# fschmid56/EfficientAT

Hardware: NVIDIA H100
Metric: clips/sec (10s@32kHz) mn10_as fwd+bwd (higher is better)
Workload: dtype f32

## Files before the change

efficientat_b200/csrc/pw_tma.cu:

```cuda
#include <cstdlib>

#include "tma_common.cuh"

namespace {
using namespace tc;
using namespace tma;

constexpr int BM = 128;
constexpr int BN_MAX = 128;
constexpr int A_TILE = BM * 128;
constexpr int kThreads = 416;
constexpr int kFirstCons = 4, kTmaWarp = 12, kConsThreads = 256;
constexpr int STG_BYTES = 16 * 128;

struct TmaParams {
  int M, N, K;
  int BN, n_tiles, m_tiles, k_blocks, r_blocks;
  int bnp;
  int stages, wres;
  int stg_bufs;
  int wpre;
  int n_samples, tps, tile_rps;
  int wdyn;
  uint32_t stage_bytes, off_w, off_stg, off_f, off_bar;
  int kpad;
  const float* in_scale; const float* in_shift; const float* gate; int in_act; int rps;
  const float* scale; const float* shift;
  double* stat_sum; double* stat_sq;
};

template <int NP>
__device__ __forceinline__ void mma_pieces(float (&d)[NP][16], uint64_t da, uint64_t db) {
#pragma unroll
  for (int pc = 0; pc < NP; ++pc) wgmma_n32<0, 0>(d[pc], da, db + (uint64_t)(pc * 256));
}

template <int EPI, int XACT, int NP>
__global__ void __launch_bounds__(kThreads, 1)
pw_tma_kernel(const __grid_constant__ CUtensorMap mapA, const __grid_constant__ CUtensorMap mapW,
              const __grid_constant__ CUtensorMap mapC, const __grid_constant__ CUtensorMap mapR, const TmaParams p) {
  extern __shared__ __align__(1024) unsigned char smem[];
  unsigned char* s_w = smem + p.off_w;
  unsigned char* s_stg = smem + p.off_stg;
  float* s_isc = reinterpret_cast<float*>(smem + p.off_f);
  float* s_ish = s_isc + p.kpad;
  float* s_shift = s_ish + p.kpad;
  float* s_stat = s_shift + p.bnp;
  uint64_t* bars = reinterpret_cast<uint64_t*>(smem + p.off_bar);
  const int S = p.stages;
  const uint32_t bar_full = smem_u32(bars), bar_ready = bar_full + 8 * S, bar_empty = bar_ready + 8 * S;
  const uint32_t bar_wfull = bar_empty + 8 * S;

  const int warp = threadIdx.x >> 5, lane = threadIdx.x & 31;
  if (threadIdx.x == 0) {
    for (int s = 0; s < S; ++s) { mbar_init(bar_full + 8 * s, 1); mbar_init(bar_ready + 8 * s, 4); mbar_init(bar_empty + 8 * s, 2); }
    mbar_init(bar_wfull, 1);
    asm volatile("fence.mbarrier_init.release.cluster;" ::: "memory");
    asm volatile("prefetch.tensormap [%0];" ::"l"(reinterpret_cast<uint64_t>(&mapA)) : "memory");
    asm volatile("prefetch.tensormap [%0];" ::"l"(reinterpret_cast<uint64_t>(&mapW)) : "memory");
    asm volatile("prefetch.tensormap [%0];" ::"l"(reinterpret_cast<uint64_t>(&mapC)) : "memory");
  }
  if (XACT >= 0) {
    for (int i = threadIdx.x; i < p.kpad; i += kThreads) {
      s_isc[i] = i < p.K ? p.in_scale[i] : 0.f;
      s_ish[i] = i < p.K ? p.in_shift[i] : 0.f;
    }
  }
  for (int i = threadIdx.x; i < 16 * p.bnp; i += kThreads) s_stat[i] = 0.f;
  fence_proxy_async();
  __syncthreads();

  const int total_tiles = p.m_tiles * p.n_tiles;
  constexpr int BN = 32 * NP;
  const int kb_total = p.k_blocks + p.r_blocks;
  const uint32_t w_tile = (uint32_t)BN * 128u;
  const uint32_t stage_base = smem_u32(smem);
  int nt = blockIdx.x / p.m_tiles, mt = blockIdx.x - nt * p.m_tiles;
  auto next_tile = [&]() { mt += gridDim.x; while (mt >= p.m_tiles) { mt -= p.m_tiles; ++nt; } };
  auto split_tile = [&](int m, int& bs, int& jt) { if (p.n_samples == 1) { bs = 0; jt = m; } else { bs = m / p.tps; jt = m - bs * p.tps; } };

  if (warp == kTmaWarp) {
    if (lane == 0) {
      int s = 0, s_prev = 0, cur_nt = -1;
      uint32_t ph = 0, ph_prev = 0;
      bool first = true;
      for (int t = blockIdx.x; t < total_tiles; t += gridDim.x) {
        int bs, jt;
        split_tile(mt, bs, jt);
        const int m0 = jt * BM, n0 = nt * BN;
        const int wb = p.wdyn ? bs : 0;
        const int wkey = nt * p.n_samples + wb;
        if (p.wres && wkey != cur_nt) {
          if (!first) mbar_wait(bar_empty + 8 * s_prev, ph_prev);
          mbar_expect_tx(bar_wfull, (uint32_t)p.k_blocks * w_tile);
          for (int kb = 0; kb < p.k_blocks; ++kb)
            tma_load_3d(&mapW, bar_wfull, smem_u32(s_w) + (uint32_t)kb * w_tile, kb * (p.wpre ? 2 * KB : KB), n0, wb);
          cur_nt = wkey;
        }
        next_tile();
        for (int kb = 0; kb < kb_total; ++kb) {
          mbar_wait(bar_empty + 8 * s, ph ^ 1u);
          const uint32_t dst = stage_base + (uint32_t)s * p.stage_bytes;
          if (kb < p.k_blocks) {
            mbar_expect_tx(bar_full + 8 * s, A_TILE + (p.wres ? 0u : w_tile));
            tma_load_3d(&mapA, bar_full + 8 * s, dst, kb * KB, m0, bs);
            if (!p.wres) tma_load_3d(&mapW, bar_full + 8 * s, dst + A_TILE, kb * (p.wpre ? 2 * KB : KB), n0, wb);
          } else {
            mbar_expect_tx(bar_full + 8 * s, A_TILE);
            tma_load_3d(&mapR, bar_full + 8 * s, dst, n0 + (kb - p.k_blocks) * KB, m0, bs);
          }
          s_prev = s; ph_prev = ph; first = false;
          if (++s == S) { s = 0; ph ^= 1u; }
        }
      }
    }
    __syncwarp();
  } else if (warp < kFirstCons) {
    const int ft = threadIdx.x;
    int s = 0, cur_nt = -1;
    uint32_t ph = 0, wphase = 0;
    const bool fold = EPI != 0 && p.scale != nullptr;
    auto do_fix_w = [&](unsigned char* w, int kb, int n0) {
      const int lg = pair_lg(p.K - kb * KB);
      if (fold) {
        if (lg == 2) fix_w<2, true>(w, ft, BN, p.scale, n0, p.N);
        else fix_w<1, true>(w, ft, BN, p.scale, n0, p.N);
      } else {
        if (lg == 2) fix_w<2, false>(w, ft, BN, nullptr, n0, p.N);
        else fix_w<1, false>(w, ft, BN, nullptr, n0, p.N);
      }
    };
    for (int t = blockIdx.x; t < total_tiles; t += gridDim.x) {
      int bs, jt;
      split_tile(mt, bs, jt);
      const int n0 = nt * BN;
      const int rows_valid = min(BM, p.tile_rps - jt * BM);
      const int wkey = nt * p.n_samples + (p.wdyn ? bs : 0);
      if (p.wres && wkey != cur_nt) {
        mbar_wait(bar_wfull, wphase);
        wphase ^= 1u;
        if (!p.wpre)
          for (int kb = 0; kb < p.k_blocks; ++kb) do_fix_w(s_w + (size_t)kb * w_tile, kb, n0);
        cur_nt = wkey;
      }
      next_tile();
      int b0 = 0, off0 = 0;
      if (p.gate != nullptr) { const int m0 = bs * p.tile_rps + jt * BM; b0 = m0 / p.rps; off0 = m0 - b0 * p.rps; }
      for (int kb = 0; kb < kb_total; ++kb) {
        mbar_wait(bar_full + 8 * s, ph);
        unsigned char* tile = smem + (size_t)s * p.stage_bytes;
        if (kb >= p.k_blocks) {
          fix_a<2, -1>(tile, ft, BM, nullptr, nullptr, 0, nullptr, 0, 0, 1, 0);
        } else {
          const int lg = pair_lg(p.K - kb * KB);
          const int k = kb * KB + (ft & ((1 << lg) - 1)) * 8;
          if (lg == 2) fix_a<2, XACT>(tile, ft, rows_valid, s_isc, s_ish, k, p.gate, off0, b0, p.rps, p.K);
          else fix_a<1, XACT>(tile, ft, rows_valid, s_isc, s_ish, k, p.gate, off0, b0, p.rps, p.K);
          if (!p.wres && !p.wpre) do_fix_w(tile + A_TILE, kb, n0);
        }
        fence_proxy_async();
        __syncwarp();
        if (lane == 0) mbar_arrive(bar_ready + 8 * s);
        if (++s == S) { s = 0; ph ^= 1u; }
      }
    }
  } else {
    const int cw = warp - kFirstCons;
    const int g = cw >> 2;
    const int wq = cw & 3;
    const int ctid = threadIdx.x - kFirstCons * 32;
    unsigned char* stg = s_stg + (size_t)cw * p.stg_bufs * STG_BYTES;
    const int bnp = p.bnp;
    float* my_stat = s_stat + cw * 2 * bnp;
    const bool do_stats = EPI == 0 && p.stat_sum != nullptr;
    const uint64_t desc0 = gmma_desc(0);
    const uint64_t wres0 = desc0 + (smem_u32(s_w) >> 4);
    const uint32_t w_tile16 = w_tile >> 4;
    float csum[NP], csq[NP];
#pragma unroll
    for (int c = 0; c < NP; ++c) { csum[c] = 0.f; csq[c] = 0.f; }
    int cur_nt = -1, cb = 0, s = 0;
    uint32_t ph = 0;
    auto flush_stats = [&](int nt_old) {
#pragma unroll
      for (int c = 0; c < NP; ++c) { my_stat[c * 32 + lane] = csum[c]; my_stat[bnp + c * 32 + lane] = csq[c]; csum[c] = 0.f; csq[c] = 0.f; }
      asm volatile("bar.sync 1, 256;" ::: "memory");
      for (int e = ctid; e < BN; e += kConsThreads) {
        const int n = nt_old * BN + e;
        float a = 0.f, b = 0.f;
#pragma unroll
        for (int w = 0; w < 8; ++w) { a += s_stat[w * 2 * bnp + e]; b += s_stat[w * 2 * bnp + bnp + e]; }
        if (n < p.N) { atomicAdd(p.stat_sum + n, (double)a); atomicAdd(p.stat_sq + n, (double)b); }
      }
      asm volatile("bar.sync 1, 256;" ::: "memory");
    };
    for (int t = blockIdx.x; t < total_tiles; t += gridDim.x) {
      int bs, jt;
      split_tile(mt, bs, jt);
      const int m0 = jt * BM, n0 = nt * BN;
      if (nt != cur_nt) {
        if (do_stats && cur_nt >= 0) flush_stats(cur_nt);
        if (EPI != 0) {
          asm volatile("bar.sync 2, 256;" ::: "memory");
          for (int e = ctid; e < BN; e += kConsThreads) s_shift[e] = (p.shift != nullptr && n0 + e < p.N) ? p.shift[n0 + e] : 0.f;
          asm volatile("bar.sync 2, 256;" ::: "memory");
        }
        cur_nt = nt;
      }
      next_tile();
      float acc[NP][16];
#pragma unroll
      for (int c = 0; c < NP; ++c)
#pragma unroll
        for (int i = 0; i < 16; ++i) acc[c][i] = 0.f;
      int pend = -1;
      auto release = [&](int st) {
        asm volatile("bar.sync %0, 128;" ::"r"(3 + g) : "memory");
        if (ctid == g * 128) mbar_arrive(bar_empty + 8 * st);
      };
      const int fr = lane >> 2, fc = 2 * (lane & 3);
      for (int kb = 0; kb < kb_total; ++kb) {
        mbar_wait(bar_ready + 8 * s, ph);
        const uint32_t sa = stage_base + (uint32_t)s * p.stage_bytes;
        if (kb < p.k_blocks) {
          const uint64_t a_hi = desc0 + ((sa + (uint32_t)g * 8192u) >> 4), a_lo = a_hi + 4;
          const uint64_t w_hi = p.wres ? wres0 + (uint32_t)kb * w_tile16 : desc0 + ((sa + A_TILE) >> 4);
          const uint64_t w_lo = w_hi + 4;
          wgmma_fence();
#pragma unroll
          for (int j = 0; j < 2; ++j) {
            const uint64_t ko = (uint64_t)(j * 2);
            mma_pieces<NP>(acc, a_hi + ko, w_hi + ko);
            mma_pieces<NP>(acc, a_lo + ko, w_hi + ko);
            mma_pieces<NP>(acc, a_hi + ko, w_lo + ko);
          }
          wgmma_commit();
          wgmma_wait<1>();
          if (pend >= 0) release(pend);
          pend = s;
        } else {
          wgmma_wait<0>();
#pragma unroll
          for (int c = 0; c < NP; ++c) wgmma_fence_regs(acc[c]);
          if (pend >= 0) { release(pend); pend = -1; }
          const int jr = kb - p.k_blocks;
          const unsigned char* tile = smem + (size_t)s * p.stage_bytes;
          const int r0 = g * 64 + wq * 16 + fr;
#pragma unroll
          for (int c = 0; c < NP; ++c) {
            if (c == jr) {
#pragma unroll
              for (int j = 0; j < 4; ++j) {
#pragma unroll
                for (int h = 0; h < 2; ++h) {
                  const int r = r0 + 8 * h;
                  const uint32_t e = (uint32_t)fc * 2;
                  const __nv_bfloat162 hi = *reinterpret_cast<const __nv_bfloat162*>(tile + swz(r, j) + e);
                  const __nv_bfloat162 lo = *reinterpret_cast<const __nv_bfloat162*>(tile + swz(r, 4 + j) + e);
                  const float2 fh = __bfloat1622float2(hi), fl = __bfloat1622float2(lo);
                  acc[c][4 * j + 2 * h] += fh.x + fl.x;
                  acc[c][4 * j + 2 * h + 1] += fh.y + fl.y;
                }
              }
            }
          }
          release(s);
        }
        if (++s == S) { s = 0; ph ^= 1u; }
      }
      if (pend >= 0) {
        wgmma_wait<0>();
        release(pend);
      }
#pragma unroll
      for (int c = 0; c < NP; ++c) wgmma_fence_regs(acc[c]);
      const int row0 = m0 + g * 64 + wq * 16;
      const int rows_left = min(16, p.tile_rps - row0);
#pragma unroll
      for (int c = 0; c < NP; ++c) {
        if (c * 32 < BN && n0 + c * 32 < p.N) {
          unsigned char* buf = stg + (size_t)cb * STG_BYTES;
          if (p.stg_bufs == 2) { cb ^= 1; if (lane == 0) tma_wait_read<1>(); }
          else if (lane == 0) tma_wait_read<0>();
          __syncwarp();
#pragma unroll
          for (int j = 0; j < 4; ++j) {
            const int cc = 8 * j + fc;
            float2 v0 = make_float2(acc[c][4 * j], acc[c][4 * j + 1]), v1 = make_float2(acc[c][4 * j + 2], acc[c][4 * j + 3]);
            if (EPI != 0) {
              const float2 sh = *reinterpret_cast<const float2*>(s_shift + c * 32 + cc);
              v0.x = act_out<EPI>(v0.x + sh.x); v0.y = act_out<EPI>(v0.y + sh.y);
              v1.x = act_out<EPI>(v1.x + sh.x); v1.y = act_out<EPI>(v1.y + sh.y);
            }
            const uint32_t co = (uint32_t)(((cc >> 2) << 4) + (cc & 3) * 4);
            *reinterpret_cast<float2*>(buf + fr * 128 + (co ^ ((fr & 7) << 4))) = v0;
            *reinterpret_cast<float2*>(buf + (fr + 8) * 128 + (co ^ (((fr + 8) & 7) << 4))) = v1;
          }
          if (do_stats) {
            __syncwarp();
            float s1 = 0.f, s2 = 0.f;
            const int cj = lane >> 2, ci = lane & 3;
            for (int r = 0; r < rows_left; ++r) {
              const float x = *reinterpret_cast<const float*>(buf + r * 128 + ((cj ^ (r & 7)) << 4) + ci * 4);
              s1 += x; s2 = fmaf(x, x, s2);
            }
            csum[c] += s1; csq[c] += s2;
          }
          fence_proxy_async();
          __syncwarp();
          if (lane == 0 && rows_left > 0) { tma_store_3d(&mapC, smem_u32(buf), n0 + c * 32, row0, bs); tma_commit(); }
        }
      }
    }
    if (do_stats && cur_nt >= 0) flush_stats(cur_nt);
    if (lane == 0) tma_wait_read<0>();
    __syncwarp();
  }
  __syncthreads();
}

__global__ void w_split_kernel(const float* __restrict__ W, const float* __restrict__ row_scale, int trans,
                               uint4* __restrict__ out, int N, int K, int k_blocks) {
  const long long items = (long long)N * k_blocks * 4;
  for (long long i = (long long)blockIdx.x * blockDim.x + threadIdx.x; i < items; i += (long long)gridDim.x * blockDim.x) {
    const int cp = (int)(i & 3);
    const long long t = i >> 2;
    const int kb = (int)(t % k_blocks), n = (int)(t / k_blocks);
    const int k0 = kb * KB + cp * 8;
    float v[8];
    const float sc = row_scale != nullptr ? __ldg(row_scale + n) : 1.f;
#pragma unroll
    for (int j = 0; j < 8; ++j) {
      const int k = k0 + j;
      v[j] = k < K ? __ldg(trans ? W + (size_t)k * N + n : W + (size_t)n * K + k) * sc : 0.f;
    }
    uint4 hi, lo;
    split8(make_float4(v[0], v[1], v[2], v[3]), make_float4(v[4], v[5], v[6], v[7]), hi, lo);
    uint4* row = out + ((size_t)n * k_blocks + kb) * 8;
    row[cp] = hi;
    row[4 + cp] = lo;
  }
}

__global__ void w_mix_split_kernel(const float* __restrict__ W, const float* __restrict__ att, int dyn_k,
                                   const float* __restrict__ row_scale, int trans, uint4* __restrict__ out, int B, int N,
                                   int K, int k_blocks) {
  const long long per = (long long)N * k_blocks * 4;
  const long long items = per * B;
  const size_t bank = (size_t)N * K;
  for (long long i = (long long)blockIdx.x * blockDim.x + threadIdx.x; i < items; i += (long long)gridDim.x * blockDim.x) {
    const int b = (int)(i / per);
    const long long r = i - (long long)b * per;
    const int cp = (int)(r & 3);
    const long long t = r >> 2;
    const int kb = (int)(t % k_blocks), n = (int)(t / k_blocks);
    const int k0 = kb * KB + cp * 8;
    float a[4] = {0.f, 0.f, 0.f, 0.f};
    for (int j = 0; j < dyn_k; ++j) a[j] = __ldg(att + (size_t)b * dyn_k + j);
    const float sc = row_scale != nullptr ? __ldg(row_scale + n) : 1.f;
    float v[8];
#pragma unroll
    for (int e = 0; e < 8; ++e) {
      const int k = k0 + e;
      float acc = 0.f;
      if (k < K) {
        const size_t off = trans ? (size_t)k * N + n : (size_t)n * K + k;
        for (int j = 0; j < dyn_k; ++j) acc = fmaf(a[j], __ldg(W + j * bank + off), acc);
      }
      v[e] = acc * sc;
    }
    uint4 hi, lo;
    split8(make_float4(v[0], v[1], v[2], v[3]), make_float4(v[4], v[5], v[6], v[7]), hi, lo);
    uint4* row = out + (((size_t)b * N + n) * k_blocks + kb) * 8;
    row[cp] = hi;
    row[4 + cp] = lo;
  }
}

int make_map_bf16(CUtensorMap* map, const void* ptr, long long rows, long long cols, int box_rows) {
  EncodeTiledFn enc = encode_fn();
  if (enc == nullptr) { eat_set_error("pw_tma: cuTensorMapEncodeTiled is not available from this driver"); return EAT_ERR_CUDA; }
  cuuint64_t gdim[2] = {(cuuint64_t)cols, (cuuint64_t)rows};
  cuuint64_t gstride[1] = {(cuuint64_t)cols * 2};
  cuuint32_t box[2] = {64, (cuuint32_t)box_rows};
  cuuint32_t estr[2] = {1, 1};
  CUresult r = enc(map, CU_TENSOR_MAP_DATA_TYPE_BFLOAT16, 2, const_cast<void*>(ptr), gdim, gstride, box, estr,
                   CU_TENSOR_MAP_INTERLEAVE_NONE, CU_TENSOR_MAP_SWIZZLE_128B, CU_TENSOR_MAP_L2_PROMOTION_L2_128B,
                   CU_TENSOR_MAP_FLOAT_OOB_FILL_NONE);
  if (r != CUDA_SUCCESS) { eat_set_error("pw_tma: cuTensorMapEncodeTiled (bf16) failed"); return EAT_ERR_CUDA; }
  return EAT_OK;
}

constexpr size_t kSmemLimit = 227 * 1024;

template <int EPI, int XACT, int NP>
int launch_kernel(const CUtensorMap& mA, const CUtensorMap& mW, const CUtensorMap& mC, const CUtensorMap& mR, const TmaParams& p,
                  size_t smem, int tiles, cudaStream_t st) {
  static unsigned long long attr_mask = 0;
  if (int rc = eat_opt_in_smem(pw_tma_kernel<EPI, XACT, NP>, kSmemLimit, attr_mask)) return rc;
  int dev = 0, sms = kNumSMs;
  cudaGetDevice(&dev);
  cudaDeviceGetAttribute(&sms, cudaDevAttrMultiProcessorCount, dev);
  pw_tma_kernel<EPI, XACT, NP><<<tiles < sms ? tiles : sms, kThreads, smem, st>>>(mA, mW, mC, mR, p);
  EAT_CHECK_LAUNCH();
  return EAT_OK;
}

struct WeightWs { int trans; void* ws; size_t bytes; const float* att; int dyn_k; };

template <int EPI, int XACT>
int launch_tma(const void* A, const float* W, void* C, const void* R, TmaParams p, cudaStream_t st, WeightWs ws) {
  int bn_max = BN_MAX;
  if (const char* e = getenv("EAT_TMA_BNMAX")) { const int v = atoi(e); if (v == 64 || v == BN_MAX) bn_max = v; }
  if (p.N <= bn_max) { p.BN = p.N <= 32 ? 32 : (p.N <= 64 ? 64 : 128); p.n_tiles = 1; }
  else {
    int best = 0; long long best_cost = 0;
    for (int bn = 64; bn <= bn_max; bn *= 2) {
      const long long nt = ceil_div(p.N, bn);
      const long long cost = nt * 72 * 1024 + nt * bn * 320;
      if (best == 0 || cost < best_cost || (cost == best_cost && bn > best)) { best = bn; best_cost = cost; }
    }
    p.BN = best; p.n_tiles = ceil_div(p.N, best);
  }
  p.bnp = 128;
  if (p.n_samples < 1) { p.n_samples = 1; p.tile_rps = p.M; }
  p.tps = ceil_div(p.tile_rps, BM);
  p.m_tiles = p.n_samples * p.tps;
  p.k_blocks = ceil_div(p.K, KB);
  p.r_blocks = R != nullptr ? ceil_div(min(p.BN, p.N), 32) : 0;
  p.kpad = XACT >= 0 ? p.k_blocks * KB : 0;
  const size_t w_tile = (size_t)p.BN * 128;
  const size_t w_res = (size_t)p.k_blocks * w_tile;
  const size_t floats = (2 * (size_t)p.kpad + 17 * (size_t)p.bnp) * 4;
  const size_t barsz = (3 * 8 + 1) * 8 + 16;
  p.stg_bufs = 2;
  const size_t fixed = (size_t)p.stg_bufs * 8 * STG_BYTES + floats + barsz + 1024 ;
  p.wres = (fixed + w_res + 4 * (size_t)A_TILE <= kSmemLimit) ? 1 : 0;
  p.stage_bytes = (uint32_t)(A_TILE + (p.wres ? 0 : w_tile));
  const size_t avail = kSmemLimit - fixed - (p.wres ? w_res : 0);
  p.stages = (int)(avail / p.stage_bytes);
  if (p.stages > 8) p.stages = 8;
  if (p.stages < 2) { eat_set_error("pw_tma: shared-memory budget exceeded (K too large for the in-transform tables)"); return EAT_ERR_UNSUPPORTED; }
  size_t off = (size_t)p.stages * p.stage_bytes;
  p.off_w = (uint32_t)off; off += p.wres ? w_res : 0;
  p.off_stg = (uint32_t)off; off += (size_t)p.stg_bufs * 8 * STG_BYTES;
  p.off_f = (uint32_t)off; off += floats;
  off = (off + 7) & ~(size_t)7;
  p.off_bar = (uint32_t)off; off += (3 * (size_t)p.stages + 1) * 8 + 16;
  const size_t smem = off;
  if (smem > kSmemLimit) { eat_set_error("pw_tma: shared-memory carve-up exceeds its budget"); return EAT_ERR_UNSUPPORTED; }
  CUtensorMap mA, mW, mC, mR;
  const long long ns = p.n_samples, rps = p.tile_rps;
  if (int rc = make_map3(&mA, A, ns, rps, p.K, BM, 4)) return rc;
  p.wpre = 0;
  p.wdyn = 0;
  if (ws.ws != nullptr) {
    const long long wsamples = ws.att != nullptr ? ns : 1;
    const size_t need = (size_t)wsamples * p.N * p.k_blocks * 128;
    if (ws.bytes < need || (((uintptr_t)ws.ws) & 127)) { eat_set_error("pw_tma: weight workspace too small or not 128-byte aligned"); return EAT_ERR_ARG; }
    const long long items = wsamples * p.N * p.k_blocks * 4;
    const int grid = (int)min((long long)kNumSMs * 8, ceil_div_ll(items, 256));
    const float* fold = (EPI != 0) ? p.scale : nullptr;
    if (ws.att != nullptr) {
      w_mix_split_kernel<<<grid, 256, 0, st>>>(W, ws.att, ws.dyn_k, fold, ws.trans, reinterpret_cast<uint4*>(ws.ws), (int)ns, p.N, p.K, p.k_blocks);
      p.wdyn = 1;
    } else {
      w_split_kernel<<<grid, 256, 0, st>>>(W, fold, ws.trans, reinterpret_cast<uint4*>(ws.ws), p.N, p.K, p.k_blocks);
    }
    EAT_CHECK_LAUNCH();
    p.wpre = 1;
    if (int rc = make_map3(&mW, ws.ws, wsamples, p.N, (long long)p.k_blocks * 64, p.BN, 2)) return rc;
  } else {
    if (ws.trans || ws.att != nullptr) { eat_set_error("pw_tma: transposed / per-sample weights need the weight workspace"); return EAT_ERR_ARG; }
    if (int rc = make_map3(&mW, W, 1, p.N, p.K, p.BN, 4)) return rc;
  }
  if (int rc = make_map3(&mC, C, ns, rps, p.N, 16, 4)) return rc;
  if (int rc = make_map3(&mR, R != nullptr ? R : C, ns, rps, p.N, BM, 4)) return rc;
  const int tiles = p.m_tiles * p.n_tiles;
  if (p.BN == 32) return launch_kernel<EPI, XACT, 1>(mA, mW, mC, mR, p, smem, tiles, st);
  if (p.BN == 64) return launch_kernel<EPI, XACT, 2>(mA, mW, mC, mR, p, smem, tiles, st);
  return launch_kernel<EPI, XACT, 4>(mA, mW, mC, mR, p, smem, tiles, st);
}

template <int EPI>
int launch_tma_x(const void* A, const float* W, void* C, const void* R, const TmaParams& p, cudaStream_t st, WeightWs ws) {
  if (p.in_scale == nullptr) return launch_tma<EPI, -1>(A, W, C, R, p, st, ws);
  if (p.in_act == EAT_ACT_RELU) return launch_tma<EPI, 1>(A, W, C, R, p, st, ws);
  if (p.in_act == EAT_ACT_HSWISH) return launch_tma<EPI, 2>(A, W, C, R, p, st, ws);
  return launch_tma<EPI, 0>(A, W, C, R, p, st, ws);
}

}

extern "C" int eat_pw_tma_fwd(const float* A, const float* W, int w_trans, float* C, long long M, int N, int K,
                              const float* in_scale, const float* in_shift, int in_act, const float* gate,
                              int rows_per_sample, const float* scale, const float* shift, int act, const float* residual,
                              double* stat_sum, double* stat_sq, void* w_ws, long long w_ws_bytes, cudaStream_t st) {
  if (M == 0) return EAT_OK;
  if (act == EAT_ACT_SIGMOID || in_act == EAT_ACT_SIGMOID) { eat_set_error("pw_tma: sigmoid epilogues run on the CUDA-core GEMM (eat_gemm_simt_fwd)"); return EAT_ERR_UNSUPPORTED; }
  const bool aff = scale != nullptr || shift != nullptr || act != 0;
  if (residual != nullptr && act != EAT_ACT_NONE) { eat_set_error("pw_tma: the residual is accumulated before the activation; residual + activation is not offered"); return EAT_ERR_UNSUPPORTED; }
  if (stat_sum != nullptr && (aff || residual != nullptr)) {
    eat_set_error("pw_tma: batch statistics are produced by the raw-output variant only (no affine/activation/residual)");
    return EAT_ERR_UNSUPPORTED;
  }
  if ((in_scale == nullptr) != (in_shift == nullptr)) { eat_set_error("pw_tma: in_scale and in_shift come together"); return EAT_ERR_ARG; }
  if (K % 4 != 0 || N % 4 != 0) { eat_set_error("pw_tma: K and N must be multiples of 4 (16-byte row pitch for TMA)"); return EAT_ERR_ARG; }
  if (M >= (1ll << 31) - BM) { eat_set_error("pw_tma: M too large"); return EAT_ERR_ARG; }
  if ((((uintptr_t)A) | ((uintptr_t)W) | ((uintptr_t)C) | ((uintptr_t)residual) | ((uintptr_t)gate)) & 15) { eat_set_error("pw_tma: operands must be 16-byte aligned"); return EAT_ERR_ARG; }
  TmaParams p{};
  p.M = (int)M; p.N = N; p.K = K;
  p.in_scale = in_scale; p.in_shift = in_shift; p.gate = gate; p.in_act = in_act; p.rps = rows_per_sample > 0 ? rows_per_sample : 1;
  p.scale = scale; p.shift = shift; p.stat_sum = stat_sum; p.stat_sq = stat_sq;
  const WeightWs ws{w_trans, w_ws, (size_t)(w_ws_bytes > 0 ? w_ws_bytes : 0), nullptr, 0};
  if (!aff) return launch_tma_x<0>(A, W, C, residual, p, st, ws);
  if (act == EAT_ACT_RELU) return launch_tma_x<2>(A, W, C, residual, p, st, ws);
  if (act == EAT_ACT_HSWISH) return launch_tma_x<3>(A, W, C, residual, p, st, ws);
  return launch_tma_x<1>(A, W, C, residual, p, st, ws);
}

extern "C" int eat_pw_tma_dyn_fwd(const float* A, const float* W, const float* att, int dyn_k, int w_trans, float* C,
                                  long long M, int N, int K, int rows_per_sample, const float* scale, const float* shift,
                                  int act, const float* residual, double* stat_sum, double* stat_sq, void* w_ws,
                                  long long w_ws_bytes, cudaStream_t st) {
  if (M == 0) return EAT_OK;
  if (dyn_k < 1 || dyn_k > 4) { eat_set_error("pw_tma_dyn: 1..4 kernels supported"); return EAT_ERR_UNSUPPORTED; }
  if (rows_per_sample < 1 || M % rows_per_sample != 0) { eat_set_error("pw_tma_dyn: M must be B * rows_per_sample"); return EAT_ERR_ARG; }
  if (act == EAT_ACT_SIGMOID) { eat_set_error("pw_tma_dyn: sigmoid epilogue is not offered"); return EAT_ERR_UNSUPPORTED; }
  const bool aff = scale != nullptr || shift != nullptr || act != 0;
  if (residual != nullptr && act != EAT_ACT_NONE) { eat_set_error("pw_tma_dyn: residual + activation is not offered"); return EAT_ERR_UNSUPPORTED; }
  if (stat_sum != nullptr && (aff || residual != nullptr)) { eat_set_error("pw_tma_dyn: statistics come from the raw-output variant only"); return EAT_ERR_UNSUPPORTED; }
  if (K % 4 != 0 || N % 4 != 0) { eat_set_error("pw_tma_dyn: K and N must be multiples of 4"); return EAT_ERR_ARG; }
  if (M >= (1ll << 31) - BM) { eat_set_error("pw_tma_dyn: M too large"); return EAT_ERR_ARG; }
  if (w_ws == nullptr || att == nullptr) { eat_set_error("pw_tma_dyn: attention weights and the weight workspace are required"); return EAT_ERR_ARG; }
  if ((((uintptr_t)A) | ((uintptr_t)W) | ((uintptr_t)C) | ((uintptr_t)residual)) & 15) { eat_set_error("pw_tma_dyn: operands must be 16-byte aligned"); return EAT_ERR_ARG; }
  TmaParams p{};
  p.M = (int)M; p.N = N; p.K = K;
  p.rps = 1;
  p.scale = scale; p.shift = shift; p.stat_sum = stat_sum; p.stat_sq = stat_sq;
  p.n_samples = (int)(M / rows_per_sample); p.tile_rps = rows_per_sample;
  const WeightWs ws{w_trans, w_ws, (size_t)(w_ws_bytes > 0 ? w_ws_bytes : 0), att, dyn_k};
  if (!aff) return launch_tma_x<0>(A, W, C, residual, p, st, ws);
  if (act == EAT_ACT_RELU) return launch_tma_x<2>(A, W, C, residual, p, st, ws);
  if (act == EAT_ACT_HSWISH) return launch_tma_x<3>(A, W, C, residual, p, st, ws);
  return launch_tma_x<1>(A, W, C, residual, p, st, ws);
}
```

efficientat_b200/csrc/tc_common.cuh:

```cuda
#pragma once
#include "common.cuh"

namespace tc {

__device__ __forceinline__ uint32_t smem_u32(const void* p) { return (uint32_t)__cvta_generic_to_shared(p); }

__device__ __forceinline__ void mbar_init(uint32_t bar, uint32_t count) {
  asm volatile("mbarrier.init.shared::cta.b64 [%0], %1;" ::"r"(bar), "r"(count));
}
__device__ __forceinline__ void mbar_arrive(uint32_t bar) {
  asm volatile("mbarrier.arrive.shared::cta.b64 _, [%0];" ::"r"(bar) : "memory");
}
__device__ __forceinline__ void mbar_wait(uint32_t bar, uint32_t parity) {
  asm volatile(
      "{\n"
      ".reg .pred P1;\n"
      "LAB_WAIT:\n"
      "mbarrier.try_wait.parity.shared::cta.b64 P1, [%0], %1, %2;\n"
      "@P1 bra DONE;\n"
      "bra LAB_WAIT;\n"
      "DONE:\n"
      "}\n" ::"r"(bar), "r"(parity), "r"(0x989680) : "memory");
}
__device__ __forceinline__ void l2_prefetch(const void* p, uint32_t bytes) {
  asm volatile("cp.async.bulk.prefetch.L2.global [%0], %1;" ::"l"(p), "r"(bytes) : "memory");
}
__device__ __forceinline__ void fence_proxy_async() { asm volatile("fence.proxy.async.shared::cta;" ::: "memory"); }

__device__ __forceinline__ uint64_t gmma_desc(uint32_t saddr, uint32_t lbo_bytes = 16, uint32_t sbo_bytes = 1024) {
  uint64_t d = (uint64_t)((saddr & 0x3FFFF) >> 4);
  d |= (uint64_t)((lbo_bytes >> 4) & 0x3FFF) << 16;
  d |= (uint64_t)((sbo_bytes >> 4) & 0x3FFF) << 32;
  d |= (uint64_t)1 << 62;
  return d;
}
__device__ __forceinline__ void wgmma_fence() { asm volatile("wgmma.fence.sync.aligned;" ::: "memory"); }
__device__ __forceinline__ void wgmma_commit() { asm volatile("wgmma.commit_group.sync.aligned;" ::: "memory"); }
template <int N> __device__ __forceinline__ void wgmma_wait() { asm volatile("wgmma.wait_group.sync.aligned %0;" ::"n"(N) : "memory"); }
template <int R> __device__ __forceinline__ void wgmma_fence_regs(float (&d)[R]) {
#pragma unroll
  for (int i = 0; i < R; ++i) asm volatile("" : "+f"(d[i])::"memory");
}
template <int TA, int TB>
__device__ __forceinline__ void wgmma_n16(float (&d)[8], uint64_t da, uint64_t db) {
  asm volatile(
      "{\n.reg .pred p;\nsetp.ne.b32 p, %10, 0;\n"
      "wgmma.mma_async.sync.aligned.m64n16k16.f32.bf16.bf16 {%0, %1, %2, %3, %4, %5, %6, %7}, %8, %9, p, 1, 1, %11, %12;\n}\n"
      : "+f"(d[0]), "+f"(d[1]), "+f"(d[2]), "+f"(d[3]), "+f"(d[4]), "+f"(d[5]), "+f"(d[6]), "+f"(d[7])
      : "l"(da), "l"(db), "r"(1), "n"(TA), "n"(TB));
}
template <int TA, int TB>
__device__ __forceinline__ void wgmma_n32(float (&d)[16], uint64_t da, uint64_t db) {
  asm volatile(
      "{\n.reg .pred p;\nsetp.ne.b32 p, %18, 0;\n"
      "wgmma.mma_async.sync.aligned.m64n32k16.f32.bf16.bf16 {%0, %1, %2, %3, %4, %5, %6, %7, %8, %9, %10, %11, %12, %13, %14, %15}, %16, %17, p, 1, 1, %19, %20;\n}\n"
      : "+f"(d[0]), "+f"(d[1]), "+f"(d[2]), "+f"(d[3]), "+f"(d[4]), "+f"(d[5]), "+f"(d[6]), "+f"(d[7]), "+f"(d[8]), "+f"(d[9]), "+f"(d[10]), "+f"(d[11]), "+f"(d[12]), "+f"(d[13]), "+f"(d[14]), "+f"(d[15])
      : "l"(da), "l"(db), "r"(1), "n"(TA), "n"(TB));
}
template <int TA, int TB>
__device__ __forceinline__ void wgmma_n64(float (&d)[32], uint64_t da, uint64_t db) {
  asm volatile(
      "{\n.reg .pred p;\nsetp.ne.b32 p, %34, 0;\n"
      "wgmma.mma_async.sync.aligned.m64n64k16.f32.bf16.bf16 {%0, %1, %2, %3, %4, %5, %6, %7, %8, %9, %10, %11, %12, %13, %14, %15, %16, %17, %18, %19, %20, %21, %22, %23, %24, %25, %26, %27, %28, %29, %30, %31}, %32, %33, p, 1, 1, %35, %36;\n}\n"
      : "+f"(d[0]), "+f"(d[1]), "+f"(d[2]), "+f"(d[3]), "+f"(d[4]), "+f"(d[5]), "+f"(d[6]), "+f"(d[7]), "+f"(d[8]), "+f"(d[9]), "+f"(d[10]), "+f"(d[11]), "+f"(d[12]), "+f"(d[13]), "+f"(d[14]), "+f"(d[15]), "+f"(d[16]), "+f"(d[17]), "+f"(d[18]), "+f"(d[19]), "+f"(d[20]), "+f"(d[21]), "+f"(d[22]), "+f"(d[23]), "+f"(d[24]), "+f"(d[25]), "+f"(d[26]), "+f"(d[27]), "+f"(d[28]), "+f"(d[29]), "+f"(d[30]), "+f"(d[31])
      : "l"(da), "l"(db), "r"(1), "n"(TA), "n"(TB));
}

__device__ __forceinline__ uint32_t swz(int row, int chunk) {
  return (uint32_t)((row >> 3) * 1024 + (row & 7) * 128 + ((chunk ^ (row & 7)) << 4));
}

__device__ __forceinline__ uint32_t pack_bf16(float a, float b) {
  __nv_bfloat162 h = __floats2bfloat162_rn(a, b);
  return *reinterpret_cast<uint32_t*>(&h);
}

template <int NP>
__device__ __forceinline__ void store_chunk(unsigned char* hi_tile, unsigned char* lo_tile, uint32_t off, const float (&v)[8]) {
  uint4 h;
  h.x = pack_bf16(v[0], v[1]); h.y = pack_bf16(v[2], v[3]); h.z = pack_bf16(v[4], v[5]); h.w = pack_bf16(v[6], v[7]);
  *reinterpret_cast<uint4*>(hi_tile + off) = h;
  if (NP == 2) {
    float r[8];
    const __nv_bfloat162* hh = reinterpret_cast<const __nv_bfloat162*>(&h);
#pragma unroll
    for (int i = 0; i < 4; ++i) {
      float2 f = __bfloat1622float2(hh[i]);
      r[2 * i] = v[2 * i] - f.x;
      r[2 * i + 1] = v[2 * i + 1] - f.y;
    }
    uint4 l;
    l.x = pack_bf16(r[0], r[1]); l.y = pack_bf16(r[2], r[3]); l.z = pack_bf16(r[4], r[5]); l.w = pack_bf16(r[6], r[7]);
    *reinterpret_cast<uint4*>(lo_tile + off) = l;
  }
}

template <typename T>
__device__ __forceinline__ void load_chunk(const T* p, float (&v)[8]);
template <>
__device__ __forceinline__ void load_chunk<float>(const float* p, float (&v)[8]) {
  float4 a = __ldg(reinterpret_cast<const float4*>(p)), b = __ldg(reinterpret_cast<const float4*>(p) + 1);
  v[0] = a.x; v[1] = a.y; v[2] = a.z; v[3] = a.w; v[4] = b.x; v[5] = b.y; v[6] = b.z; v[7] = b.w;
}
template <>
__device__ __forceinline__ void load_chunk<__nv_bfloat16>(const __nv_bfloat16* p, float (&v)[8]) {
  uint4 t = __ldg(reinterpret_cast<const uint4*>(p));
  const __nv_bfloat162* h = reinterpret_cast<const __nv_bfloat162*>(&t);
#pragma unroll
  for (int i = 0; i < 4; ++i) { float2 f = __bfloat1622float2(h[i]); v[2 * i] = f.x; v[2 * i + 1] = f.y; }
}


}
```

Baseline: 5152.

## Fit pointwise GEMM tile width to N in multiples of 8 with single wgmma

```diff
diff --git a/efficientat_b200/csrc/pw_tma.cu b/efficientat_b200/csrc/pw_tma.cu
--- a/efficientat_b200/csrc/pw_tma.cu
+++ b/efficientat_b200/csrc/pw_tma.cu
@@ -1,4 +1,5 @@
-#include <cstdlib>
+#include <type_traits>
+#include <utility>
 
 #include "tma_common.cuh"
 
@@ -29,16 +30,13 @@
   double* stat_sum; double* stat_sq;
 };
 
-template <int NP>
-__device__ __forceinline__ void mma_pieces(float (&d)[NP][16], uint64_t da, uint64_t db) {
-#pragma unroll
-  for (int pc = 0; pc < NP; ++pc) wgmma_n32<0, 0>(d[pc], da, db + (uint64_t)(pc * 256));
-}
-
-template <int EPI, int XACT, int NP>
+template <int EPI, int XACT, int BN>
 __global__ void __launch_bounds__(kThreads, 1)
 pw_tma_kernel(const __grid_constant__ CUtensorMap mapA, const __grid_constant__ CUtensorMap mapW,
-              const __grid_constant__ CUtensorMap mapC, const __grid_constant__ CUtensorMap mapR, const TmaParams p) {
+              const __grid_constant__ CUtensorMap mapC, const __grid_constant__ CUtensorMap mapCt,
+              const __grid_constant__ CUtensorMap mapR, const TmaParams p) {
+  constexpr int NC = (BN + 31) / 32;
+  constexpr int TAIL = BN % 32;
   extern __shared__ __align__(1024) unsigned char smem[];
   unsigned char* s_w = smem + p.off_w;
   unsigned char* s_stg = smem + p.off_stg;
@@ -59,6 +57,7 @@
     asm volatile("prefetch.tensormap [%0];" ::"l"(reinterpret_cast<uint64_t>(&mapA)) : "memory");
     asm volatile("prefetch.tensormap [%0];" ::"l"(reinterpret_cast<uint64_t>(&mapW)) : "memory");
     asm volatile("prefetch.tensormap [%0];" ::"l"(reinterpret_cast<uint64_t>(&mapC)) : "memory");
+    if (TAIL != 0) asm volatile("prefetch.tensormap [%0];" ::"l"(reinterpret_cast<uint64_t>(&mapCt)) : "memory");
   }
   if (XACT >= 0) {
     for (int i = threadIdx.x; i < p.kpad; i += kThreads) {
@@ -71,12 +70,13 @@
   __syncthreads();
 
   const int total_tiles = p.m_tiles * p.n_tiles;
-  constexpr int BN = 32 * NP;
   const int kb_total = p.k_blocks + p.r_blocks;
   const uint32_t w_tile = (uint32_t)BN * 128u;
   const uint32_t stage_base = smem_u32(smem);
-  int nt = blockIdx.x / p.m_tiles, mt = blockIdx.x - nt * p.m_tiles;
-  auto next_tile = [&]() { mt += gridDim.x; while (mt >= p.m_tiles) { mt -= p.m_tiles; ++nt; } };
+  const int cpn = gridDim.x / p.n_tiles;
+  const int nt = blockIdx.x % p.n_tiles;
+  int mt = blockIdx.x / p.n_tiles;
+  auto next_tile = [&]() { mt += cpn; };
   auto split_tile = [&](int m, int& bs, int& jt) { if (p.n_samples == 1) { bs = 0; jt = m; } else { bs = m / p.tps; jt = m - bs * p.tps; } };
 
   if (warp == kTmaWarp) {
@@ -176,14 +176,14 @@
     const uint64_t desc0 = gmma_desc(0);
     const uint64_t wres0 = desc0 + (smem_u32(s_w) >> 4);
     const uint32_t w_tile16 = w_tile >> 4;
-    float csum[NP], csq[NP];
-#pragma unroll
-    for (int c = 0; c < NP; ++c) { csum[c] = 0.f; csq[c] = 0.f; }
+    float csum[NC], csq[NC];
+#pragma unroll
+    for (int c = 0; c < NC; ++c) { csum[c] = 0.f; csq[c] = 0.f; }
     int cur_nt = -1, cb = 0, s = 0;
     uint32_t ph = 0;
     auto flush_stats = [&](int nt_old) {
 #pragma unroll
-      for (int c = 0; c < NP; ++c) { my_stat[c * 32 + lane] = csum[c]; my_stat[bnp + c * 32 + lane] = csq[c]; csum[c] = 0.f; csq[c] = 0.f; }
+      for (int c = 0; c < NC; ++c) { my_stat[c * 32 + lane] = csum[c]; my_stat[bnp + c * 32 + lane] = csq[c]; csum[c] = 0.f; csq[c] = 0.f; }
       asm volatile("bar.sync 1, 256;" ::: "memory");
       for (int e = ctid; e < BN; e += kConsThreads) {
         const int n = nt_old * BN + e;
@@ -208,11 +208,9 @@
         cur_nt = nt;
       }
       next_tile();
-      float acc[NP][16];
-#pragma unroll
-      for (int c = 0; c < NP; ++c)
-#pragma unroll
-        for (int i = 0; i < 16; ++i) acc[c][i] = 0.f;
+      float acc[BN / 2];
+#pragma unroll
+      for (int i = 0; i < BN / 2; ++i) acc[i] = 0.f;
       int pend = -1;
       auto release = [&](int st) {
         asm volatile("bar.sync %0, 128;" ::"r"(3 + g) : "memory");
@@ -230,9 +228,9 @@
 #pragma unroll
           for (int j = 0; j < 2; ++j) {
             const uint64_t ko = (uint64_t)(j * 2);
-            mma_pieces<NP>(acc, a_hi + ko, w_hi + ko);
-            mma_pieces<NP>(acc, a_lo + ko, w_hi + ko);
-            mma_pieces<NP>(acc, a_hi + ko, w_lo + ko);
+            wgmma_kk<BN>(acc, a_hi + ko, w_hi + ko);
+            wgmma_kk<BN>(acc, a_lo + ko, w_hi + ko);
+            wgmma_kk<BN>(acc, a_hi + ko, w_lo + ko);
           }
           wgmma_commit();
           wgmma_wait<1>();
@@ -240,26 +238,27 @@
           pend = s;
         } else {
           wgmma_wait<0>();
-#pragma unroll
-          for (int c = 0; c < NP; ++c) wgmma_fence_regs(acc[c]);
+          wgmma_fence_regs(acc);
           if (pend >= 0) { release(pend); pend = -1; }
           const int jr = kb - p.k_blocks;
           const unsigned char* tile = smem + (size_t)s * p.stage_bytes;
           const int r0 = g * 64 + wq * 16 + fr;
 #pragma unroll
-          for (int c = 0; c < NP; ++c) {
+          for (int c = 0; c < NC; ++c) {
             if (c == jr) {
 #pragma unroll
               for (int j = 0; j < 4; ++j) {
-#pragma unroll
-                for (int h = 0; h < 2; ++h) {
-                  const int r = r0 + 8 * h;
-                  const uint32_t e = (uint32_t)fc * 2;
-                  const __nv_bfloat162 hi = *reinterpret_cast<const __nv_bfloat162*>(tile + swz(r, j) + e);
-                  const __nv_bfloat162 lo = *reinterpret_cast<const __nv_bfloat162*>(tile + swz(r, 4 + j) + e);
-                  const float2 fh = __bfloat1622float2(hi), fl = __bfloat1622float2(lo);
-                  acc[c][4 * j + 2 * h] += fh.x + fl.x;
-                  acc[c][4 * j + 2 * h + 1] += fh.y + fl.y;
+                if (32 * c + 8 * j < BN) {
+#pragma unroll
+                  for (int h = 0; h < 2; ++h) {
+                    const int r = r0 + 8 * h;
+                    const uint32_t e = (uint32_t)fc * 2;
+                    const __nv_bfloat162 hi = *reinterpret_cast<const __nv_bfloat162*>(tile + swz(r, j) + e);
+                    const __nv_bfloat162 lo = *reinterpret_cast<const __nv_bfloat162*>(tile + swz(r, 4 + j) + e);
+                    const float2 fh = __bfloat1622float2(hi), fl = __bfloat1622float2(lo);
+                    acc[16 * c + 4 * j + 2 * h] += fh.x + fl.x;
+                    acc[16 * c + 4 * j + 2 * h + 1] += fh.y + fl.y;
+                  }
                 }
               }
             }
@@ -272,43 +271,55 @@
         wgmma_wait<0>();
         release(pend);
       }
-#pragma unroll
-      for (int c = 0; c < NP; ++c) wgmma_fence_regs(acc[c]);
+      wgmma_fence_regs(acc);
       const int row0 = m0 + g * 64 + wq * 16;
       const int rows_left = min(16, p.tile_rps - row0);
 #pragma unroll
-      for (int c = 0; c < NP; ++c) {
-        if (c * 32 < BN && n0 + c * 32 < p.N) {
+      for (int c = 0; c < NC; ++c) {
+        const int cw = (TAIL != 0 && c == NC - 1) ? TAIL : 32;
+        const bool tail = cw < 32 && n0 + BN < p.N;
+        if (n0 + c * 32 < p.N) {
           unsigned char* buf = stg + (size_t)cb * STG_BYTES;
           if (p.stg_bufs == 2) { cb ^= 1; if (lane == 0) tma_wait_read<1>(); }
           else if (lane == 0) tma_wait_read<0>();
           __syncwarp();
 #pragma unroll
           for (int j = 0; j < 4; ++j) {
-            const int cc = 8 * j + fc;
-            float2 v0 = make_float2(acc[c][4 * j], acc[c][4 * j + 1]), v1 = make_float2(acc[c][4 * j + 2], acc[c][4 * j + 3]);
-            if (EPI != 0) {
-              const float2 sh = *reinterpret_cast<const float2*>(s_shift + c * 32 + cc);
-              v0.x = act_out<EPI>(v0.x + sh.x); v0.y = act_out<EPI>(v0.y + sh.y);
-              v1.x = act_out<EPI>(v1.x + sh.x); v1.y = act_out<EPI>(v1.y + sh.y);
+            if (32 * c + 8 * j < BN) {
+              const int cc = 8 * j + fc;
+              const float* a4 = acc + 16 * c + 4 * j;
+              float2 v0 = make_float2(a4[0], a4[1]), v1 = make_float2(a4[2], a4[3]);
+              if (EPI != 0) {
+                const float2 sh = *reinterpret_cast<const float2*>(s_shift + c * 32 + cc);
+                v0.x = act_out<EPI>(v0.x + sh.x); v0.y = act_out<EPI>(v0.y + sh.y);
+                v1.x = act_out<EPI>(v1.x + sh.x); v1.y = act_out<EPI>(v1.y + sh.y);
+              }
+              if (tail) {
+                *reinterpret_cast<float2*>(buf + (fr * cw + cc) * 4) = v0;
+                *reinterpret_cast<float2*>(buf + ((fr + 8) * cw + cc) * 4) = v1;
+              } else {
+                const uint32_t co = (uint32_t)(((cc >> 2) << 4) + (cc & 3) * 4);
+                *reinterpret_cast<float2*>(buf + fr * 128 + (co ^ ((fr & 7) << 4))) = v0;
+                *reinterpret_cast<float2*>(buf + (fr + 8) * 128 + (co ^ (((fr + 8) & 7) << 4))) = v1;
+              }
             }
-            const uint32_t co = (uint32_t)(((cc >> 2) << 4) + (cc & 3) * 4);
-            *reinterpret_cast<float2*>(buf + fr * 128 + (co ^ ((fr & 7) << 4))) = v0;
-            *reinterpret_cast<float2*>(buf + (fr + 8) * 128 + (co ^ (((fr + 8) & 7) << 4))) = v1;
           }
           if (do_stats) {
             __syncwarp();
             float s1 = 0.f, s2 = 0.f;
             const int cj = lane >> 2, ci = lane & 3;
-            for (int r = 0; r < rows_left; ++r) {
-              const float x = *reinterpret_cast<const float*>(buf + r * 128 + ((cj ^ (r & 7)) << 4) + ci * 4);
-              s1 += x; s2 = fmaf(x, x, s2);
+            if (lane < cw) {
+              for (int r = 0; r < rows_left; ++r) {
+                const uint32_t o = tail ? (uint32_t)(r * cw + lane) * 4 : (uint32_t)(r * 128 + ((cj ^ (r & 7)) << 4) + ci * 4);
+                const float x = *reinterpret_cast<const float*>(buf + o);
+                s1 += x; s2 = fmaf(x, x, s2);
+              }
             }
             csum[c] += s1; csq[c] += s2;
           }
           fence_proxy_async();
           __syncwarp();
-          if (lane == 0 && rows_left > 0) { tma_store_3d(&mapC, smem_u32(buf), n0 + c * 32, row0, bs); tma_commit(); }
+          if (lane == 0 && rows_left > 0) { tma_store_3d(tail ? &mapCt : &mapC, smem_u32(buf), n0 + c * 32, row0, bs); tma_commit(); }
         }
       }
     }
@@ -391,38 +402,65 @@
   return EAT_OK;
 }
 
+int make_map_tail(CUtensorMap* map, const void* ptr, long long samples, long long rows, long long cols, int cw) {
+  EncodeTiledFn enc = encode_fn();
+  if (enc == nullptr) { eat_set_error("pw_tma: cuTensorMapEncodeTiled is not available from this driver"); return EAT_ERR_CUDA; }
+  cuuint64_t gdim[3] = {(cuuint64_t)cols, (cuuint64_t)rows, (cuuint64_t)samples};
+  cuuint64_t gstride[2] = {(cuuint64_t)cols * 4, (cuuint64_t)(rows * cols * 4)};
+  cuuint32_t box[3] = {(cuuint32_t)cw, 16, 1};
+  cuuint32_t estr[3] = {1, 1, 1};
+  CUresult r = enc(map, CU_TENSOR_MAP_DATA_TYPE_FLOAT32, 3, const_cast<void*>(ptr), gdim, gstride, box, estr,
+                   CU_TENSOR_MAP_INTERLEAVE_NONE, CU_TENSOR_MAP_SWIZZLE_NONE, CU_TENSOR_MAP_L2_PROMOTION_L2_128B,
+                   CU_TENSOR_MAP_FLOAT_OOB_FILL_NONE);
+  if (r != CUDA_SUCCESS) { eat_set_error("pw_tma: cuTensorMapEncodeTiled (tail store) failed"); return EAT_ERR_CUDA; }
+  return EAT_OK;
+}
+
 constexpr size_t kSmemLimit = 227 * 1024;
 
-template <int EPI, int XACT, int NP>
-int launch_kernel(const CUtensorMap& mA, const CUtensorMap& mW, const CUtensorMap& mC, const CUtensorMap& mR, const TmaParams& p,
-                  size_t smem, int tiles, cudaStream_t st) {
+struct Maps { CUtensorMap A, W, C, Ct, R; };
+
+template <int EPI, int XACT, int BN>
+int launch_kernel(const Maps& m, const TmaParams& p, size_t smem, int tiles, cudaStream_t st) {
   static unsigned long long attr_mask = 0;
-  if (int rc = eat_opt_in_smem(pw_tma_kernel<EPI, XACT, NP>, kSmemLimit, attr_mask)) return rc;
+  if (int rc = eat_opt_in_smem(pw_tma_kernel<EPI, XACT, BN>, kSmemLimit, attr_mask)) return rc;
   int dev = 0, sms = kNumSMs;
   cudaGetDevice(&dev);
   cudaDeviceGetAttribute(&sms, cudaDevAttrMultiProcessorCount, dev);
-  pw_tma_kernel<EPI, XACT, NP><<<tiles < sms ? tiles : sms, kThreads, smem, st>>>(mA, mW, mC, mR, p);
+  const int grid = min(tiles, max(p.n_tiles, sms / p.n_tiles * p.n_tiles));
+  pw_tma_kernel<EPI, XACT, BN><<<grid, kThreads, smem, st>>>(m.A, m.W, m.C, m.Ct, m.R, p);
   EAT_CHECK_LAUNCH();
   return EAT_OK;
 }
 
+template <int EPI>
+using Widths = std::conditional_t<EPI == 0,
+                                  std::integer_sequence<int, 8, 16, 24, 32, 40, 48, 56, 64, 72, 80, 88, 96, 104, 112, 120, 128>,
+                                  std::integer_sequence<int, 32, 64, 128>>;
+
+template <int... W>
+constexpr int fit_width(std::integer_sequence<int, W...>, int bn) {
+  int best = BN_MAX;
+  for (int w : {W...}) if (w >= bn && w < best) best = w;
+  return best;
+}
+
+template <int EPI, int XACT, int... W>
+int launch_width(std::integer_sequence<int, W...>, const Maps& m, const TmaParams& p, size_t smem, int tiles, cudaStream_t st) {
+  int rc = EAT_ERR_UNSUPPORTED;
+  const bool found = ((p.BN == W && (rc = launch_kernel<EPI, XACT, W>(m, p, smem, tiles, st), true)) || ...);
+  if (!found) eat_set_error("pw_tma: no kernel for this tile width");
+  return rc;
+}
+
 struct WeightWs { int trans; void* ws; size_t bytes; const float* att; int dyn_k; };
 
 template <int EPI, int XACT>
 int launch_tma(const void* A, const float* W, void* C, const void* R, TmaParams p, cudaStream_t st, WeightWs ws) {
-  int bn_max = BN_MAX;
-  if (const char* e = getenv("EAT_TMA_BNMAX")) { const int v = atoi(e); if (v == 64 || v == BN_MAX) bn_max = v; }
-  if (p.N <= bn_max) { p.BN = p.N <= 32 ? 32 : (p.N <= 64 ? 64 : 128); p.n_tiles = 1; }
-  else {
-    int best = 0; long long best_cost = 0;
-    for (int bn = 64; bn <= bn_max; bn *= 2) {
-      const long long nt = ceil_div(p.N, bn);
-      const long long cost = nt * 72 * 1024 + nt * bn * 320;
-      if (best == 0 || cost < best_cost || (cost == best_cost && bn > best)) { best = bn; best_cost = cost; }
-    }
-    p.BN = best; p.n_tiles = ceil_div(p.N, best);
-  }
-  p.bnp = 128;
+  p.n_tiles = ceil_div(p.N, BN_MAX);
+  p.BN = fit_width(Widths<EPI>{}, (ceil_div(p.N, p.n_tiles) + 7) & ~7);
+  p.n_tiles = ceil_div(p.N, p.BN);
+  p.bnp = BN_MAX;
   if (p.n_samples < 1) { p.n_samples = 1; p.tile_rps = p.M; }
   p.tps = ceil_div(p.tile_rps, BM);
   p.m_tiles = p.n_samples * p.tps;
@@ -449,7 +487,8 @@
   p.off_bar = (uint32_t)off; off += (3 * (size_t)p.stages + 1) * 8 + 16;
   const size_t smem = off;
   if (smem > kSmemLimit) { eat_set_error("pw_tma: shared-memory carve-up exceeds its budget"); return EAT_ERR_UNSUPPORTED; }
-  CUtensorMap mA, mW, mC, mR;
+  Maps m;
+  CUtensorMap &mA = m.A, &mW = m.W, &mC = m.C, &mR = m.R;
   const long long ns = p.n_samples, rps = p.tile_rps;
   if (int rc = make_map3(&mA, A, ns, rps, p.K, BM, 4)) return rc;
   p.wpre = 0;
@@ -475,11 +514,13 @@
     if (int rc = make_map3(&mW, W, 1, p.N, p.K, p.BN, 4)) return rc;
   }
   if (int rc = make_map3(&mC, C, ns, rps, p.N, 16, 4)) return rc;
+  if (p.n_tiles > 1 && p.BN % 32 != 0) {
+    if (int rc = make_map_tail(&m.Ct, C, ns, rps, p.N, p.BN % 32)) return rc;
+  } else {
+    m.Ct = mC;
+  }
   if (int rc = make_map3(&mR, R != nullptr ? R : C, ns, rps, p.N, BM, 4)) return rc;
-  const int tiles = p.m_tiles * p.n_tiles;
-  if (p.BN == 32) return launch_kernel<EPI, XACT, 1>(mA, mW, mC, mR, p, smem, tiles, st);
-  if (p.BN == 64) return launch_kernel<EPI, XACT, 2>(mA, mW, mC, mR, p, smem, tiles, st);
-  return launch_kernel<EPI, XACT, 4>(mA, mW, mC, mR, p, smem, tiles, st);
+  return launch_width<EPI, XACT>(Widths<EPI>{}, m, p, smem, p.m_tiles * p.n_tiles, st);
 }
 
 template <int EPI>
diff --git a/efficientat_b200/csrc/tc_common.cuh b/efficientat_b200/csrc/tc_common.cuh
--- a/efficientat_b200/csrc/tc_common.cuh
+++ b/efficientat_b200/csrc/tc_common.cuh
@@ -66,6 +66,53 @@
       : "l"(da), "l"(db), "r"(1), "n"(TA), "n"(TB));
 }
 
+#define EAT_WG_S8 "%0, %1, %2, %3"
+#define EAT_WG_S16 EAT_WG_S8 ", %4, %5, %6, %7"
+#define EAT_WG_S24 EAT_WG_S16 ", %8, %9, %10, %11"
+#define EAT_WG_S32 EAT_WG_S24 ", %12, %13, %14, %15"
+#define EAT_WG_S40 EAT_WG_S32 ", %16, %17, %18, %19"
+#define EAT_WG_S48 EAT_WG_S40 ", %20, %21, %22, %23"
+#define EAT_WG_S56 EAT_WG_S48 ", %24, %25, %26, %27"
+#define EAT_WG_S64 EAT_WG_S56 ", %28, %29, %30, %31"
+#define EAT_WG_S72 EAT_WG_S64 ", %32, %33, %34, %35"
+#define EAT_WG_S80 EAT_WG_S72 ", %36, %37, %38, %39"
+#define EAT_WG_S88 EAT_WG_S80 ", %40, %41, %42, %43"
+#define EAT_WG_S96 EAT_WG_S88 ", %44, %45, %46, %47"
+#define EAT_WG_S104 EAT_WG_S96 ", %48, %49, %50, %51"
+#define EAT_WG_S112 EAT_WG_S104 ", %52, %53, %54, %55"
+#define EAT_WG_S120 EAT_WG_S112 ", %56, %57, %58, %59"
+#define EAT_WG_S128 EAT_WG_S120 ", %60, %61, %62, %63"
+#define EAT_WG_O8 "+f"(d[0]), "+f"(d[1]), "+f"(d[2]), "+f"(d[3])
+#define EAT_WG_O16 EAT_WG_O8, "+f"(d[4]), "+f"(d[5]), "+f"(d[6]), "+f"(d[7])
+#define EAT_WG_O24 EAT_WG_O16, "+f"(d[8]), "+f"(d[9]), "+f"(d[10]), "+f"(d[11])
+#define EAT_WG_O32 EAT_WG_O24, "+f"(d[12]), "+f"(d[13]), "+f"(d[14]), "+f"(d[15])
+#define EAT_WG_O40 EAT_WG_O32, "+f"(d[16]), "+f"(d[17]), "+f"(d[18]), "+f"(d[19])
+#define EAT_WG_O48 EAT_WG_O40, "+f"(d[20]), "+f"(d[21]), "+f"(d[22]), "+f"(d[23])
+#define EAT_WG_O56 EAT_WG_O48, "+f"(d[24]), "+f"(d[25]), "+f"(d[26]), "+f"(d[27])
+#define EAT_WG_O64 EAT_WG_O56, "+f"(d[28]), "+f"(d[29]), "+f"(d[30]), "+f"(d[31])
+#define EAT_WG_O72 EAT_WG_O64, "+f"(d[32]), "+f"(d[33]), "+f"(d[34]), "+f"(d[35])
+#define EAT_WG_O80 EAT_WG_O72, "+f"(d[36]), "+f"(d[37]), "+f"(d[38]), "+f"(d[39])
+#define EAT_WG_O88 EAT_WG_O80, "+f"(d[40]), "+f"(d[41]), "+f"(d[42]), "+f"(d[43])
+#define EAT_WG_O96 EAT_WG_O88, "+f"(d[44]), "+f"(d[45]), "+f"(d[46]), "+f"(d[47])
+#define EAT_WG_O104 EAT_WG_O96, "+f"(d[48]), "+f"(d[49]), "+f"(d[50]), "+f"(d[51])
+#define EAT_WG_O112 EAT_WG_O104, "+f"(d[52]), "+f"(d[53]), "+f"(d[54]), "+f"(d[55])
+#define EAT_WG_O120 EAT_WG_O112, "+f"(d[56]), "+f"(d[57]), "+f"(d[58]), "+f"(d[59])
+#define EAT_WG_O128 EAT_WG_O120, "+f"(d[60]), "+f"(d[61]), "+f"(d[62]), "+f"(d[63])
+#define EAT_WG_CASE(W, DA, DB, ONE)                                                                                     \
+  if constexpr (N == W)                                                                                                 \
+    asm volatile("{\n.reg .pred p;\nsetp.ne.b32 p, %" #ONE ", 0;\n"                                                     \
+                 "wgmma.mma_async.sync.aligned.m64n" #W "k16.f32.bf16.bf16 {" EAT_WG_S##W "}, %" #DA ", %" #DB ", p, 1, 1, 0, 0;\n}\n" \
+                 : EAT_WG_O##W : "l"(da), "l"(db), "r"(1));
+template <int N>
+__device__ __forceinline__ void wgmma_kk(float (&d)[N / 2], uint64_t da, uint64_t db) {
+  static_assert(N % 8 == 0 && N >= 8 && N <= 128, "m64nNk16: N is a multiple of 8 up to 128 here");
+  EAT_WG_CASE(8, 4, 5, 6) EAT_WG_CASE(16, 8, 9, 10) EAT_WG_CASE(24, 12, 13, 14) EAT_WG_CASE(32, 16, 17, 18)
+  EAT_WG_CASE(40, 20, 21, 22) EAT_WG_CASE(48, 24, 25, 26) EAT_WG_CASE(56, 28, 29, 30) EAT_WG_CASE(64, 32, 33, 34)
+  EAT_WG_CASE(72, 36, 37, 38) EAT_WG_CASE(80, 40, 41, 42) EAT_WG_CASE(88, 44, 45, 46) EAT_WG_CASE(96, 48, 49, 50)
+  EAT_WG_CASE(104, 52, 53, 54) EAT_WG_CASE(112, 56, 57, 58) EAT_WG_CASE(120, 60, 61, 62) EAT_WG_CASE(128, 64, 65, 66)
+}
+#undef EAT_WG_CASE
+
 __device__ __forceinline__ uint32_t swz(int row, int chunk) {
   return (uint32_t)((row >> 3) * 1024 + (row & 7) * 128 + ((chunk ^ (row & 7)) << 4));
 }
```

After: 5359 (median of 6 runs). +4.0%, better.
